# RubensBenevides/Point-Cloud-Registration-with-Global-Refinement

Measured on AMD Instinct MI355X. Metric: point-cloud pairs registered/sec (200k pts, 3 GICP scales), higher is better.
Workload: dtype f32 points+search, f64 normal equations (SURVEY 8a fp column)

## Files before the change

point-cloud-registration-with-global-refinement_amd/csrc/pcr_api.hip:

```cpp
#include <cmath>
#include <cstring>
#include <cstdlib>
#include <cstdio>
#include <atomic>
#include <mutex>
#include <thread>
#include <vector>
#include "pcr_octree.h"

extern "C" int pcr_version(void) { return 220; }

PcrOptions &pcr_options() {
    static PcrOptions o;
    static std::once_flag once;
    std::call_once(once, []() {
        if (const char *e = getenv("PCR_KNN_WAVE")) o.knn_wave = atoi(e);
        if (const char *e = getenv("PCR_KNNW_BUDGET")) o.knnw_budget = atoi(e);
        if (const char *e = getenv("PCR_FENCE_PREP")) o.fence_prep = atoi(e);
        if (getenv("PCR_ICP_VERIFY")) o.icp_verify = 1;
        if (const char *e = getenv("PCR_SPFH_FLOAT64")) o.spfh_float64 = atoi(e);
        if (const char *e = getenv("PCR_RADIUS_LIST_SELECT")) o.radius_list_select = atoi(e);
        if (const char *e = getenv("PCR_FEATNN_MUTUAL")) o.featnn_mutual = atoi(e);
        if (const char *e = getenv("PCR_ICP_SCALES")) o.icp_scales = atoi(e);
        if (const char *e = getenv("PCR_SEARCH_SORT_QUERIES")) o.search_sort_queries = atoi(e);
        if (const char *e = getenv("PCR_FPS_FORM")) o.fps_form = atoi(e);
        if (const char *e = getenv("PCR_FPS_WGS")) o.fps_wgs = atoi(e);
        if (const char *e = getenv("PCR_FPS_TIMEOUT")) o.fps_timeout = atoi(e);
    });
    return o;
}
PcrCounters &pcr_counters() { static PcrCounters c; return c; }
extern "C" long long pcr_counter(const char *name, int reset) {
    if (!name) return -1;
    PcrCounters &c = pcr_counters();
    std::atomic<long long> *v = !strcmp(name, "fgr_group_barrier_timeouts") ? &c.fgr_group_barrier_timeouts : !strcmp(name, "fgr_group_pool_overflows") ? &c.fgr_group_pool_overflows
                               : !strcmp(name, "fgr_group_pairs_redone_alone") ? &c.fgr_group_pairs_redone_alone : nullptr;
    if (!v) return -1;
    return reset ? v->exchange(0) : v->load();
}
extern "C" int pcr_set_option(const char *name, long long value) {
    if (!name) return PCR_EINVAL;
    PcrOptions &o = pcr_options();
    if (!strcmp(name, "knn_wave")) { o.knn_wave = (int)value; return PCR_OK; }
    if (!strcmp(name, "knnw_budget")) { o.knnw_budget = (int)value; return PCR_OK; }
    if (!strcmp(name, "fence_prep")) { o.fence_prep = (int)value; return PCR_OK; }
    if (!strcmp(name, "icp_verify")) { o.icp_verify = (int)value; return PCR_OK; }
    if (!strcmp(name, "spfh_float64")) { o.spfh_float64 = (int)value; return PCR_OK; }
    if (!strcmp(name, "radius_list_select")) { o.radius_list_select = (int)value; return PCR_OK; }
    if (!strcmp(name, "arena_poison")) { o.arena_poison = (int)value; return PCR_OK; }
    if (!strcmp(name, "featnn_mutual")) { o.featnn_mutual = (int)value; return PCR_OK; }
    if (!strcmp(name, "icp_scales")) { o.icp_scales = (int)value; return PCR_OK; }
    if (!strcmp(name, "search_sort_queries")) { o.search_sort_queries = (int)value; return PCR_OK; }
    if (!strcmp(name, "fps_form")) { o.fps_form = (int)value; return PCR_OK; }
    if (!strcmp(name, "fps_wgs")) { o.fps_wgs = (int)value; return PCR_OK; }
    if (!strcmp(name, "fps_timeout")) { o.fps_timeout = (int)value; return PCR_OK; }
    return PCR_EINVAL;
}

extern "C" int pcr_create(int device, pcr_context **out) {
    if (!out) return PCR_EINVAL;
    *out = nullptr;
    int count = 0;
    if (hipGetDeviceCount(&count) != hipSuccess || count <= 0) return PCR_EHIP;
    if (device < 0 || device >= count) return PCR_EINVAL;
    if (hipSetDevice(device) != hipSuccess) return PCR_EHIP;
    pcr_context *ctx = new pcr_context();
    ctx->device = device;
    for (int i = 0; i < 2; i++)
        if (hipEventCreateWithFlags(&ctx->side_ev[i], hipEventDisableTiming) != hipSuccess) { delete ctx; return PCR_EHIP; }
    for (int i = 0; i < 8; i++)
        if (hipEventCreateWithFlags(&ctx->lane_ev[i], hipEventDisableTiming) != hipSuccess) { delete ctx; return PCR_EHIP; }
    ctx->pinned_cap = 1 << 16;
    if (hipHostMalloc((void **)&ctx->pinned, ctx->pinned_cap, hipHostMallocDefault) != hipSuccess) { delete ctx; return PCR_EHIP; }
    for (int i = 0; i < 2; i++)
        if (hipEventCreateWithFlags(&ctx->ev[i], hipEventDisableTiming) != hipSuccess) { delete ctx; return PCR_EHIP; }
    for (int i = 0; i < 2; i++)
        if (hipEventCreateWithFlags(&ctx->fence_ev[i], hipEventDisableTiming) != hipSuccess) { delete ctx; return PCR_EHIP; }
    ctx->fence_default = true;
    *out = ctx;
    return PCR_OK;
}

extern "C" int pcr_destroy(pcr_context *ctx) {
    if (!ctx) return PCR_OK;
    (void)hipSetDevice(ctx->device);
    if (ctx->stream) (void)hipStreamSynchronize(ctx->stream);
    if (ctx->arena) (void)hipFree(ctx->arena);
    if (ctx->aux) (void)hipFree(ctx->aux);
    if (ctx->icp_group_dev) (void)hipFree(ctx->icp_group_dev);
    if (ctx->icp_group_host) (void)hipHostFree(ctx->icp_group_host);
    if (ctx->desc_dev) (void)hipFree(ctx->desc_dev);
    if (ctx->desc_host) (void)hipHostFree(ctx->desc_host);
    if (ctx->pinned) (void)hipHostFree(ctx->pinned);
    for (int i = 0; i < 2; i++) if (ctx->ev[i]) (void)hipEventDestroy(ctx->ev[i]);
    for (int i = 0; i < 2; i++) if (ctx->fence_ev[i]) (void)hipEventDestroy(ctx->fence_ev[i]);
    for (hipEvent_t e : ctx->prof_events) (void)hipEventDestroy(e);
    for (auto &g : ctx->icp_graphs) { (void)hipGraphExecDestroy(g.exec); if (g.graph) (void)hipGraphDestroy(g.graph); }
    if (ctx->own_stream) (void)hipStreamDestroy(ctx->own_stream);
    if (ctx->side_stream) { (void)hipStreamSynchronize(ctx->side_stream); (void)hipStreamDestroy(ctx->side_stream); }
    if (ctx->side_stream2) { (void)hipStreamSynchronize(ctx->side_stream2); (void)hipStreamDestroy(ctx->side_stream2); }
    for (int i = 0; i < 2; i++) if (ctx->side_ev[i]) (void)hipEventDestroy(ctx->side_ev[i]);
    for (int i = 0; i < 8; i++) if (ctx->lane_ev[i]) (void)hipEventDestroy(ctx->lane_ev[i]);
    delete ctx;
    return PCR_OK;
}

extern "C" int pcr_set_stream(pcr_context *ctx, void *s) {
    if (!ctx) return PCR_EINVAL;
    if (ctx->stream) (void)hipStreamSynchronize(ctx->stream);
    ctx->stream = s ? (hipStream_t)s : ctx->own_stream;
    ctx->fence_default = (s == nullptr);
    return PCR_OK;
}
static void use_private_stream(pcr_context *ctx) {
    if (ctx->stream) (void)hipStreamSynchronize(ctx->stream);
    ctx->stream = ctx->own_stream;
    ctx->fence_default = false;
}

extern "C" int pcr_profile_enable(pcr_context *ctx, int on) {
    if (!ctx) return PCR_EINVAL;
    ctx->profiling = on ? 1 : 0;
    return PCR_OK;
}
extern "C" int pcr_profile_read(pcr_context *ctx, double *out16, int reset) {
    if (!ctx || !out16) return PCR_EINVAL;
    for (int i = 0; i < 16; i++) { out16[i] = ctx->prof[i]; if (reset) ctx->prof[i] = 0; }
    return PCR_OK;
}

extern "C" const char *pcr_last_error(const pcr_context *ctx) { return ctx ? ctx->err.c_str() : "null context"; }

int pcr_arena_reserve(pcr_context *ctx, size_t bytes) {
    ctx->arena_off = 0;
    if (const int poison = pcr_options().arena_poison.load(std::memory_order_relaxed)) {
        if (ctx->arena) { PCR_HIP_CHECK(ctx, hipDeviceSynchronize()); PCR_HIP_CHECK(ctx, hipMemset(ctx->arena, poison & 0xff, ctx->arena_cap)); }
    }
    if (bytes <= ctx->arena_cap) return PCR_OK;
// ... 1191 lines not shown
```

point-cloud-registration-with-global-refinement_amd/csrc/pcr_cloud.hip:

```cpp
#include <cstdlib>
#include <cstring>
#include <cstdio>
#include <vector>
#include "pcr_octree.h"

#define BS 256

struct BoundsArgs { const float *xyz; int64_t n; float *part; float *out6; int nb; };
struct OpBoundsPartial : PcrOp<BoundsArgs, BS> {
    __device__ static inline void run(const BoundsArgs &a) {
        if ((int)blockIdx.x >= a.nb) return;
        float mn[3] = {3.4e38f, 3.4e38f, 3.4e38f}, mx[3] = {-3.4e38f, -3.4e38f, -3.4e38f};
        for (int64_t i = blockIdx.x * (int64_t)BS + threadIdx.x; i < a.n; i += (int64_t)a.nb * BS) {
            float x = a.xyz[i * 3], y = a.xyz[i * 3 + 1], z = a.xyz[i * 3 + 2];
            mn[0] = fminf(mn[0], x); mn[1] = fminf(mn[1], y); mn[2] = fminf(mn[2], z);
            mx[0] = fmaxf(mx[0], x); mx[1] = fmaxf(mx[1], y); mx[2] = fmaxf(mx[2], z);
        }
        __shared__ float s[BS / PCR_WAVE][6];
        const int lane = threadIdx.x & 63, w = threadIdx.x >> 6;
#pragma unroll
        for (int d = 0; d < 3; d++) { mn[d] = pcr_wave_min(mn[d]); mx[d] = pcr_wave_max(mx[d]); }
        if (lane == 0) { for (int d = 0; d < 3; d++) { s[w][d] = mn[d]; s[w][3 + d] = mx[d]; } }
        __syncthreads();
        if (threadIdx.x < 6) {
// ... 1375 lines not shown
                if ((ci & hm) == (ipre & hm)) atomicAdd(&dig[ob][(ci >> sh) & 255u], 1u);
            });
            __builtin_amdgcn_fence(__ATOMIC_RELEASE, "workgroup"); __builtin_amdgcn_wave_barrier(); __builtin_amdgcn_fence(__ATOMIC_ACQUIRE, "workgroup");
            if (act) {
                int cum = 0, b = 0;
                for (; b < 255; b++) { const int h = (int)dig[ob][b]; if (cum + h >= r2) break; cum += h; }
                r2 -= cum;
                ipre = (ipre & hm) | ((unsigned long long)b << sh);
            }
            __builtin_amdgcn_wave_barrier();
        }
        int cnt = 0;
        auto write = [&](int first, int count) {
            for (int base = first; base < first + count; base += OCT) {
                const int idx = base + ol;
                bool take = false;
                if (fix && idx < first + count) {
                    const float4 p = a.t.pts[idx];
                    const float d2 = pcr_d2(p.x - q.x, p.y - q.y, p.z - q.z);
                    if (d2 < a.r2f && d2 <= hi) {
                        if (d2 < lo || all_band) take = true;
                        else {
                            const unsigned long long kk = key_of(p);
                            take = kk < kpre || (kk == kpre && (all_ties || (unsigned long long)a.perm[idx] <= ipre));
                        }
                    }
                }
                const unsigned mask = (unsigned)(__ballot(take) >> (oct * 8)) & 0xffu;
                const int pos = cnt + __builtin_popcount(mask & ((1u << ol) - 1u));
                if (take && pos < a.k) row[pos] = idx;
                cnt += __builtin_popcount(mask);
            }
        };
        oct_search_group(a.t, m, gstk[threadIdx.x >> 6], fix, leaf0, q.x, q.y, q.z, [&]() { return wb; }, write,
                         [](int, int) { return false; }, ol);
    }
}
struct OpRadiusFix : PcrOp<RadListArgs, KNN_BS> { __device__ static inline void run(const RadListArgs &a) { d_radius_fix(a); } };
int pcr_dev_radius_lists_batch(pcr_context *ctx, const DevCloud *const *cs, const uint32_t *const *perms, int count, int k, double radius, int32_t *const *idx, int32_t *const *cnt) {
    if (count < 1) return PCR_OK;
    if (count > PCR_MAX_GROUP_BATCH) { ctx->err = "radius list batch size"; return PCR_EINVAL; }
    if (!(radius > 0) || k < 1 || k > 200) { ctx->err = "radius lists: radius <= 0 or k outside 1..200"; return PCR_EINVAL; }
    std::vector<RadListArgs> ra; std::vector<KnnArgs> ka; std::vector<int> caps;
    int *counts = arena<int>(ctx, count);
    if (!counts) return PCR_ENOMEM;
    PCR_HIP_CHECK(ctx, hipMemsetAsync(counts, 0, sizeof(int) * (size_t)count, ctx->stream));
    int mc = 0;
    for (int c = 0; c < count; c++) {
        if (cs[c]->cap <= 0) continue;
        RadListArgs r;
        r.t = oct_view(cs[c]); r.n_ptr = cs[c]->n; r.r2f = (float)(radius * radius); r.k = k; r.idx = idx[c]; r.cnt = cnt[c];
        r.over_list = arena<int>(ctx, (size_t)cs[c]->cap / OCT + 1); r.over_count = counts + c;
        r.select = pcr_options().radius_list_select.load(std::memory_order_relaxed); r.perm = perms[c];
        if (!r.over_list) return PCR_ENOMEM;
        ra.push_back(r);
        KnnArgs a; std::memset(&a, 0, sizeof a);
        a.t = r.t; a.n_ptr = cs[c]->n; a.k = k;
        knn_radius(a, PCR_SEARCH_HYBRID, radius);
        a.r2cap_f = r.r2f;
        a.dbg_idx = idx[c]; a.dbg_d2 = nullptr; a.dbg_cnt = nullptr; a.seed_span = -1;
        a.hard_piece = 1; a.hard_list = r.over_list; a.hard_count = r.over_count;
        ka.push_back(a); caps.push_back(cs[c]->cap);
        mc = cs[c]->cap > mc ? cs[c]->cap : mc;
    }
    const int m = (int)ra.size();
    if (m == 0) return PCR_OK;
    PCR_TRY(PCR_BATCH_LAUNCH(ctx, OpRadiusList, ra.data(), m, dim3((unsigned)(((size_t)mc * OCT + KNN_BS - 1) / KNN_BS), m)));
    int lg = mc / (OCT * (KNN_BS / 64) * 4); lg = lg < 8 ? 8 : (lg > 2048 ? 2048 : lg);
    const dim3 grid(lg, m);
    PCR_TRY((launch_knn_octet_slots<KNN_MODE_DEBUG, true>(ctx, ka.data(), m, k, grid)));
    PCR_TRY(PCR_BATCH_LAUNCH(ctx, OpRadiusFix, ra.data(), m, grid));
    return PCR_OK;
}

struct NflArgs {
    const float4 *pts; const int *n_ptr;
    const int32_t *lidx;
    const uint8_t *keep; const int *pos;
    int k_list, k_nrm;
    const float4 *prior; float4 *normals;
    uint8_t *todo; int *todo_count;
    int *piece_list, *piece_count;
};
__device__ static inline void d_normals_from_lists(const NflArgs &a) {
    const int n = *a.n_ptr;
    const int ol = threadIdx.x & 7, oct_id = (threadIdx.x & 63) >> 3;
    const int base = (blockIdx.x * (KNN_BS / 64) + (threadIdx.x >> 6)) * 64;
    if (base >= n) return;
    double my_cu[9] = {0, 0, 0, 0, 0, 0, 0, 0, 0}, my_c = 0;
    bool my_exact = false; int my_j = 0;
    bool piece_todo = false;
#pragma unroll 1
    for (int r = 0; r < OCT; r++) {
        const int i = base + oct_id * OCT + r;
        const bool act = i < n && a.keep[i];
        int id[4]; float d[4]; bool ok[4]; float4 pn[4];
        int lc = 0, vc = 0;
        const float4 qp = a.pts[act ? i : 0];
#pragma unroll
        for (int s = 0; s < 4; s++) {
            const int slot = ol + OCT * s;
            id[s] = (act && slot < a.k_list) ? a.lidx[(size_t)i * 32 + slot] : -1;
            pn[s] = a.pts[id[s] >= 0 ? id[s] : 0];
            d[s] = id[s] >= 0 ? pcr_d2(pn[s].x - qp.x, pn[s].y - qp.y, pn[s].z - qp.z) : -1.0f;
            ok[s] = id[s] >= 0 && a.keep[id[s]];
            lc += id[s] >= 0 ? 1 : 0; vc += ok[s] ? 1 : 0;
        }
        lc = pcr_octet_sum_i(lc); vc = pcr_octet_sum_i(vc);
        const bool exact = act && (vc >= a.k_nrm || lc < a.k_list);
        const int j = act ? a.pos[i] : 0;
        if (act && ol == 0) {
            a.todo[j] = exact ? 0 : 1;
            if (!exact) atomicAdd(a.todo_count, 1);
        }
        piece_todo = piece_todo || (act && !exact);
        int excess = exact ? vc - a.k_nrm : 0;
        while (__ballot(excess > 0) != 0ull) {
            float m = -1.0f; int ms = 0;
#pragma unroll
            for (int s = 0; s < 4; s++) if (ok[s] && d[s] > m) { m = d[s]; ms = s; }
            const float om = pcr_octet_max(m);
            const int ml = __builtin_ctz((uint32_t)(__ballot(m == om) >> (threadIdx.x & 56)) & 0xffu);
            const bool hit = excess > 0 && ol == ml;
#pragma unroll
            for (int s = 0; s < 4; s++) ok[s] = ok[s] && !(hit && s == ms);
            excess -= excess > 0 ? 1 : 0;
        }
        double cu[9] = {0, 0, 0, 0, 0, 0, 0, 0, 0}, c = 0;
#pragma unroll
        for (int s = 0; s < 4; s++) {
            if (exact && ok[s]) {
                const float4 p = pn[s];
                const double x = p.x, y = p.y, z = p.z;
                cu[0] += x; cu[1] += y; cu[2] += z;
                cu[3] += x * x; cu[4] += x * y; cu[5] += x * z; cu[6] += y * y; cu[7] += y * z; cu[8] += z * z;
                c += 1.0;
            }
        }
#pragma unroll
        for (int t = 0; t < 9; t++) cu[t] = pcr_octet_sum(cu[t]);
        c = pcr_octet_sum(c);
        if (ol == r) {
            my_exact = exact; my_j = j; my_c = c;
#pragma unroll
            for (int t = 0; t < 9; t++) my_cu[t] = cu[t];
        }
    }
    if (a.piece_list && piece_todo && ol == 0) a.piece_list[atomicAdd(a.piece_count, 1)] = base + oct_id * OCT;
    if (!my_exact) return;
    double myC[6] = {1, 0, 0, 1, 0, 1};
    if (my_c >= 3.0) {
#pragma unroll
        for (int t = 0; t < 9; t++) my_cu[t] = my_cu[t] / my_c;
        myC[0] = my_cu[3] - my_cu[0] * my_cu[0]; myC[1] = my_cu[4] - my_cu[0] * my_cu[1]; myC[2] = my_cu[5] - my_cu[0] * my_cu[2];
        myC[3] = my_cu[6] - my_cu[1] * my_cu[1]; myC[4] = my_cu[7] - my_cu[1] * my_cu[2]; myC[5] = my_cu[8] - my_cu[2] * my_cu[2];
    }
    double nv[3];
    d_fast_eigen3x3(myC, nv);
    const double nn = sqrt(nv[0] * nv[0] + nv[1] * nv[1] + nv[2] * nv[2]);
    double px = 0, py = 0, pz = 0;
    if (a.prior) { const float4 pr = a.prior[my_j]; px = pr.x; py = pr.y; pz = pr.z; }
    if (nn == 0.0 || !(nn == nn)) { if (a.prior) { nv[0] = px; nv[1] = py; nv[2] = pz; } else { nv[0] = 0; nv[1] = 0; nv[2] = 1; } }
    if (a.prior && nv[0] * px + nv[1] * py + nv[2] * pz < 0.0) { nv[0] = -nv[0]; nv[1] = -nv[1]; nv[2] = -nv[2]; }
    a.normals[my_j] = make_float4((float)nv[0], (float)nv[1], (float)nv[2], 0.0f);
}

struct OpNormalsFromLists : PcrOp<NflArgs, KNN_BS> { __device__ static inline void run(const NflArgs &a) { d_normals_from_lists(a); } };

#define SOR_STAT_BLOCKS 128
struct SorStatArgs { const double *avg; const int *n_ptr; double std_ratio; double *out3; double *partials ; unsigned int *ticket; };
__device__ static inline void d_sor_stats(const SorStatArgs &aa) {
    const double *__restrict__ avg = aa.avg; const int *__restrict__ n_ptr = aa.n_ptr; const double std_ratio = aa.std_ratio;
    double *__restrict__ out3 = aa.out3; double *__restrict__ partials = aa.partials; unsigned int *__restrict__ ticket = aa.ticket;
    __shared__ double red[16][3];
    __shared__ double rows[SOR_STAT_BLOCKS * 3];
    __shared__ int is_last;
    const int n = *n_ptr, t = threadIdx.x;
    double c = 0.0;
    for (int i = 0; i < n && i < 64; i++) { const double v = avg[i]; if (v > 0) { c = v; break; } }
    double a = 0, b = 0, cnt = 0;
    for (int i = blockIdx.x * 256 + t; i < n; i += gridDim.x * 256) { const double v = avg[i]; if (v > 0) { const double d = v - c; a += d; b += d * d; cnt += 1.0; } }
    a = pcr_row16_sum(a); b = pcr_row16_sum(b); cnt = pcr_row16_sum(cnt);
    if ((t & 15) == 0) { red[t >> 4][0] = a; red[t >> 4][1] = b; red[t >> 4][2] = cnt; }
    __syncthreads();
    if (t < 3) {
        double s = 0;
        for (int r = 0; r < 16; r++) s += red[r][t];
        __hip_atomic_store(&partials[blockIdx.x * 4 + t], s, __ATOMIC_RELAXED, __HIP_MEMORY_SCOPE_AGENT);
    }
    asm volatile("s_waitcnt vmcnt(0)" ::: "memory");
    __syncthreads();
    if (t == 0) is_last = __hip_atomic_fetch_add(ticket, 1u, __ATOMIC_RELAXED, __HIP_MEMORY_SCOPE_AGENT) == gridDim.x - 1;
    __syncthreads();
    if (!is_last) return;
    for (int e = t; e < 3 * (int)gridDim.x; e += 256) {
        const double *p = partials + (e / 3) * 4 + (e % 3);
        double v;
        asm volatile("global_load_dwordx2 %0, %1, off sc0 sc1\n\ts_waitcnt vmcnt(0)" : "=&v"(v) : "v"(p) : "memory");
        rows[e] = v;
    }
    __syncthreads();
    if (t == 0) {
        double sa = 0, sb = 0, sc = 0;
        for (int r = 0; r < (int)gridDim.x; r++) { sa += rows[3 * r]; sb += rows[3 * r + 1]; sc += rows[3 * r + 2]; }
        const double valid = sc;
        const double mean = valid > 0 ? c + sa / valid : 0.0;
        const double var = valid > 1 ? (sb - sa * sa / valid) / (valid - 1.0) : 0.0;
        const double sd = sqrt(var > 0 ? var : 0.0);
        out3[0] = mean; out3[1] = sd; out3[2] = valid > 0 ? mean + std_ratio * sd : -1.0;
        *ticket = 0u;
    }
}
struct OpSorStats : PcrOp<SorStatArgs, 256> { __device__ static inline void run(const SorStatArgs &a) { d_sor_stats(a); } };

struct CompactArgs {
    const float4 *pts, *nrm; const uint8_t *flags; const int *pos; const int *n_ptr; float4 *out_pts, *out_nrm;
    const uint64_t *keys; uint64_t *out_keys; int *cnt_in_out, *cnt_kept_out; const int *kept_n;
};
__device__ static inline void d_compact_cloud(const CompactArgs &a) {
    const int i = blockIdx.x * BS + threadIdx.x;
    if (i == 0) { if (a.cnt_in_out) *a.cnt_in_out = *a.n_ptr; if (a.cnt_kept_out) *a.cnt_kept_out = *a.kept_n; }
    if (i >= *a.n_ptr || !a.flags[i]) return;
    const int o = a.pos[i];
    a.out_pts[o] = a.pts[i];
    a.out_keys[o] = a.keys[i];
    if (a.nrm && a.out_nrm) a.out_nrm[o] = a.nrm[i];
}
struct OpCompactCloud : PcrOp<CompactArgs, BS> { __device__ static inline void run(const CompactArgs &a) { d_compact_cloud(a); } };

struct SorProblem {
    const DevCloud *in; DevCloud *out; uint8_t *keep_sorted; double *avg_sorted; const float4 *prior_out; uint8_t *todo_out; int *todo_count;
    int *cnt_in_out, *cnt_kept_out;
};
static int sor_batch(pcr_context *ctx, SorProblem *pr, int count, int nb_neighbors, double std_ratio, int normal_k, bool fallback_here) {
    if (nb_neighbors < 1 || !(std_ratio > 0.0)) { ctx->err = "nb_neighbors < 1 or std_ratio <= 0"; return PCR_EINVAL; }
    if (count < 1 || count > PCR_MAX_GROUP_BATCH) { ctx->err = "SOR batch size"; return PCR_EINVAL; }
    std::vector<KnnArgs> kbv((size_t)count), fbv((size_t)count); std::vector<SorStatArgs> sbv((size_t)count); std::vector<ScanArgs> cbv((size_t)count);
    std::vector<CompactArgs> mbv((size_t)count); std::vector<NflArgs> nbv((size_t)count);
    std::memset(kbv.data(), 0, sizeof(KnnArgs) * (size_t)count); std::memset(fbv.data(), 0, sizeof(KnnArgs) * (size_t)count);
    std::memset(sbv.data(), 0, sizeof(SorStatArgs) * (size_t)count); std::memset(cbv.data(), 0, sizeof(ScanArgs) * (size_t)count);
    std::memset(mbv.data(), 0, sizeof(CompactArgs) * (size_t)count); std::memset(nbv.data(), 0, sizeof(NflArgs) * (size_t)count);
    KnnArgs *const kb = kbv.data(), *const fb = fbv.data(); SorStatArgs *const sb = sbv.data(); ScanArgs *const cb = cbv.data();
    CompactArgs *const mb = mbv.data(); NflArgs *const nb_ = nbv.data();
    std::vector<int> capsv((size_t)count); int *caps = capsv.data(); int m = 0;
    bool any_todo = false, fuse_all = true;
    int *piece_counts = (fallback_here && normal_k > 0 && normal_k <= 32) ? arena<int>(ctx, count) : nullptr;
    if (piece_counts) PCR_HIP_CHECK(ctx, hipMemsetAsync(piece_counts, 0, sizeof(int) * (size_t)count, ctx->stream));
    for (int k = 0; k < count; k++) {
        SorProblem &q = pr[k];
        const DevCloud *in = q.in; DevCloud *out = q.out;
        for (int d = 0; d < 3; d++) { out->key_org[d] = in->key_org[d]; out->key_unit[d] = in->key_unit[d]; }
        out->voxel_lattice = in->voxel_lattice;
        if (in->cap <= 0) { PCR_HIP_CHECK(ctx, hipMemsetAsync(out->n, 0, sizeof(int), ctx->stream)); continue; }
        double *avg = q.avg_sorted ? q.avg_sorted : arena<double>(ctx, in->cap);
        double *stats3 = arena<double>(ctx, 4);
        double *stat_partials = arena<double>(ctx, SOR_STAT_BLOCKS * 4);
        unsigned int *stat_ticket = arena<unsigned int>(ctx, 1);
        uint8_t *flags = q.keep_sorted ? q.keep_sorted : arena<uint8_t>(ctx, in->cap);
        int *pos = arena<int>(ctx, in->cap);
        if (!avg || !stats3 || !stat_partials || !stat_ticket || !flags || !pos) return PCR_ENOMEM;
        const bool fuse = normal_k > 0 && q.todo_out && nb_neighbors <= 32 && normal_k <= nb_neighbors;
        const int pitch = nb_neighbors <= 32 ? 32 : 64;
        int32_t *lidx = (fuse || nb_neighbors <= 64) ? arena<int32_t>(ctx, (size_t)in->cap * pitch) : nullptr;
        if ((fuse || nb_neighbors <= 64) && !lidx) return PCR_ENOMEM;
        KnnArgs &a = kb[m];
        a.t = oct_view(in); a.n_ptr = in->n; a.k = nb_neighbors; a.avg = avg; a.list_idx = lidx; a.list_pitch = pitch;
        a.zero_a = (int *)stat_ticket; a.zero_b = (fuse && q.todo_out) ? q.todo_count : nullptr;
        a.seed_span = -1;
        knn_radius(a, PCR_SEARCH_KNN, 0);
        sb[m] = SorStatArgs{avg, in->n, std_ratio, stats3, stat_partials, stat_ticket};
        PCR_TRY(scan_args(ctx, &cb[m], flags, in->n, in->cap, pos, out->n, FlagSrc{nullptr, avg, stats3}));
        mb[m] = CompactArgs{in->pts, in->nrm, flags, pos, in->n, out->pts, out->nrm, in->keys, out->keys, q.cnt_in_out, q.cnt_kept_out, out->n};
        if (q.todo_out) {
            any_todo = true;
            if (fuse) {
                NflArgs &f = nb_[m];
                f.pts = in->pts; f.n_ptr = in->n; f.lidx = lidx; f.keep = flags; f.pos = pos; f.k_list = nb_neighbors; f.k_nrm = normal_k;
                f.prior = q.prior_out; f.normals = out->nrm_final; f.todo = q.todo_out; f.todo_count = q.todo_count;
            } else {
                fuse_all = false;
                PCR_HIP_CHECK(ctx, hipMemsetAsync(q.todo_out, 1, (size_t)in->cap, ctx->stream));
            }
            if (fallback_here && normal_k > 0) {
                KnnArgs &b = fb[m];
                b.t = oct_view(in); b.n_ptr = in->n; b.k = normal_k; b.prior = q.prior_out; b.normals = out->nrm_final; b.todo = fuse ? q.todo_out : nullptr;
                b.keep = flags; b.pos = pos; b.seed_span = -1;
                knn_radius(b, PCR_SEARCH_KNN, 0);
                if (fuse && piece_counts) {
                    int *pl = arena<int>(ctx, (size_t)in->cap / OCT + 1);
                    if (!pl) return PCR_ENOMEM;
                    nb_[m].piece_list = pl; nb_[m].piece_count = piece_counts + m;
                    b.hard_list = pl; b.hard_count = piece_counts + m; b.hard_piece = 1;
                }
            }
        } else fuse_all = false;
        caps[m] = in->cap;
        m++;
    }
    if (m == 0) return PCR_OK;
    int mc = 0;
    for (int k = 0; k < m; k++) mc = caps[k] > mc ? caps[k] : mc;
    if (m > 1 && nb_neighbors > 32) { ctx->err = "batched SOR: nb_neighbors must be <= 32"; return PCR_EINVAL; }
    PCR_TRY(launch_knn_batch<KNN_MODE_SOR>(ctx, kb, caps, m));
    PCR_TRY(PCR_BATCH_LAUNCH(ctx, OpSorStats, sb, m, dim3(SOR_STAT_BLOCKS, m)));
    PCR_TRY(flag_scan_batch(ctx, cb, m));
    PCR_TRY(PCR_BATCH_LAUNCH(ctx, OpCompactCloud, mb, m, dim3((mc + BS - 1) / BS, m)));
    if (any_todo) {
        if (fuse_all) PCR_TRY(PCR_BATCH_LAUNCH(ctx, OpNormalsFromLists, nb_, m, dim3((unsigned)(((size_t)mc + KNN_BS - 1) / KNN_BS), m)));
        else for (int k = 0; k < m; k++) if (nb_[k].pts) PCR_TRY(PCR_BATCH_LAUNCH(ctx, OpNormalsFromLists, nb_ + k, 1, dim3((unsigned)(((size_t)caps[k] + KNN_BS - 1) / KNN_BS))));
        if (fallback_here && normal_k > 0) {
            bool listed = fuse_all && piece_counts != nullptr;
            for (int k = 0; k < m; k++) listed = listed && fb[k].hard_list != nullptr;
            if (listed) {
                using Op = OpKnn<KNN_MODE_NORMALS, 4, true>;
                PCR_TRY(PCR_BATCH_LAUNCH(ctx, Op, fb, m, dim3(knn_list_grid(mc), m)));
            } else if (normal_k <= 32) PCR_TRY(launch_knn_batch<KNN_MODE_NORMALS>(ctx, fb, caps, m));
            else PCR_TRY(launch_knn_each<KNN_MODE_NORMALS>(ctx, fb, caps, m));
        }
    }
    return PCR_OK;
}

int pcr_dev_sor(pcr_context *ctx, const DevCloud *in, int nb_neighbors, double std_ratio, DevCloud *out, uint8_t *keep_sorted, double *avg_sorted,
                int normal_k, const float4 *prior_out, uint8_t *todo_out, int *todo_count, int *cnt_in_out, int *cnt_kept_out, bool fallback_here) {
    ArenaMark mark(ctx);
    SorProblem p{in, out, keep_sorted, avg_sorted, prior_out, todo_out, todo_count, cnt_in_out, cnt_kept_out};
    return sor_batch(ctx, &p, 1, nb_neighbors, std_ratio, normal_k, fallback_here);
}
int pcr_dev_sor_batch(pcr_context *ctx, const DevCloud *const *ins, DevCloud *const *outs, int count, int nb_neighbors, double std_ratio, int normal_k,
                      const float4 *const *priors, uint8_t *const *todos, int *const *todo_counts, int *const *cnt_in, int *const *cnt_kept, bool fallback_here) {
    if (count > PCR_MAX_GROUP_BATCH) { ctx->err = "SOR batch size"; return PCR_EINVAL; }
    std::vector<SorProblem> pv((size_t)(count > 0 ? count : 1)); SorProblem *p = pv.data();
    for (int k = 0; k < count; k++) p[k] = SorProblem{ins[k], outs[k], nullptr, nullptr, priors ? priors[k] : nullptr, todos[k], todo_counts[k], cnt_in ? cnt_in[k] : nullptr, cnt_kept ? cnt_kept[k] : nullptr};
    return sor_batch(ctx, p, count, nb_neighbors, std_ratio, normal_k, fallback_here);
}
int pcr_dev_normals_batch(pcr_context *ctx, DevCloud *const *cs, int count, int search_kind, int knn, double radius, const float4 *const *priors, float4 *const *normals_out,
                          const uint8_t *const *todos) {
    if (search_kind != PCR_SEARCH_KNN && search_kind != PCR_SEARCH_HYBRID) { ctx->err = "normals batch: KNN or Hybrid search"; return PCR_EINVAL; }
    if (search_kind == PCR_SEARCH_HYBRID && !(radius > 0)) { ctx->err = "radius <= 0"; return PCR_EINVAL; }
    if (knn < 1) { ctx->err = "knn < 1"; return PCR_EINVAL; }
    if (count > PCR_MAX_GROUP_BATCH) { ctx->err = "normals batch size"; return PCR_EINVAL; }
    std::vector<KnnArgs> bv((size_t)(count > 0 ? count : 1)); std::memset(bv.data(), 0, sizeof(KnnArgs) * bv.size());
    KnnArgs *const b = bv.data(); std::vector<int> capsv((size_t)(count > 0 ? count : 1)); int *caps = capsv.data(); int m = 0;
    for (int k = 0; k < count; k++) {
        if (cs[k]->cap <= 0) continue;
        KnnArgs &a = b[m];
        a.t = oct_view(cs[k]); a.n_ptr = cs[k]->n; a.k = knn; a.prior = priors ? priors[k] : nullptr; a.normals = normals_out[k]; a.todo = todos ? todos[k] : nullptr; a.seed_span = -1;
        knn_radius(a, search_kind, radius);
        caps[m++] = cs[k]->cap;
    }
    if (m == 0) return PCR_OK;
    if (knn <= 32) return launch_knn_batch<KNN_MODE_NORMALS>(ctx, b, caps, m);
    return launch_knn_each<KNN_MODE_NORMALS>(ctx, b, caps, m);
}
int pcr_dev_knn_lists_batch(pcr_context *ctx, const DevCloud *const *cs, int count, int k, double radius, int32_t *const *idx, float *const *d2) {
    if (count < 1) return PCR_OK;
    if (count > PCR_MAX_GROUP_BATCH) { ctx->err = "k-NN list batch size"; return PCR_EINVAL; }
    std::vector<KnnArgs> av((size_t)count); std::memset(av.data(), 0, sizeof(KnnArgs) * av.size());
    std::vector<int> caps((size_t)count); int m = 0;
    for (int c = 0; c < count; c++) {
        if (cs[c]->cap <= 0) continue;
        KnnArgs &a = av[m];
        a.t = oct_view(cs[c]); a.n_ptr = cs[c]->n; a.k = k;
        knn_radius(a, radius > 0 ? PCR_SEARCH_HYBRID : PCR_SEARCH_KNN, radius);
        if (radius > 0) a.r2cap_f = (float)(radius * radius);
        a.dbg_idx = idx[c]; a.dbg_d2 = d2[c]; a.dbg_cnt = nullptr;
        caps[m++] = cs[c]->cap;
    }
    if (m == 0) return PCR_OK;
    return launch_knn_octet_batch<KNN_MODE_DEBUG>(ctx, av.data(), caps.data(), m);
}
int pcr_dev_flag_scan_batch(pcr_context *ctx, int count, uint8_t *const *flags, const int *const *n_ptr, const int *n_cap, int *const *pos, int *const *total_dev) {
    if (count < 1) return PCR_OK;
    std::vector<ScanArgs> a((size_t)count);
    for (int c = 0; c < count; c++) PCR_TRY(scan_args(ctx, &a[c], flags[c], n_ptr ? n_ptr[c] : nullptr, n_cap[c], pos[c], total_dev[c], FlagSrc{nullptr, nullptr, nullptr}));
    return flag_scan_batch(ctx, a.data(), count);
}

int pcr_dev_normals(pcr_context *ctx, DevCloud *c, int search_kind, int knn, double radius, const float4 *prior, float4 *normals_out, float *cov6_out,
                    const uint8_t *todo) {
    if (search_kind == PCR_SEARCH_RADIUS) {
        if (!(radius > 0)) { ctx->err = "radius <= 0"; return PCR_EINVAL; }
        if (c->cap <= 0) return PCR_OK;
        RadArgs r;
        r.t = oct_view(c); r.n_ptr = c->n; r.r2 = radius * radius; r.r2f = pcr_wide_r2f(r.r2);
        r.prior = prior; r.normals = normals_out; r.cov6 = cov6_out;
        PCR_LAUNCH(ctx, k_radius_moments, dim3((unsigned)(((size_t)c->cap * OCT + KNN_BS - 1) / KNN_BS)), dim3(KNN_BS), 0, ctx->stream, r);
        return PCR_OK;
    }
    if (knn < 1) { ctx->err = "knn < 1"; return PCR_EINVAL; }
    if (search_kind == PCR_SEARCH_HYBRID && !(radius > 0)) { ctx->err = "radius <= 0"; return PCR_EINVAL; }
    KnnArgs a = {};
// ... 10 lines not shown
```

point-cloud-registration-with-global-refinement_amd/csrc/pcr_internal.h:

```cpp
#pragma once
#include <hip/hip_runtime.h>
#include <stdint.h>
#include <string>
#include <mutex>
#include <cstring>
#include <vector>
#include <atomic>
#include "../../include/pcr_hip.h"

struct PcrOptions { std::atomic<int> knn_wave{-1}, knnw_budget{80}, fence_prep{0}, icp_verify{0}, spfh_float64{0}, radius_list_select{1}, arena_poison{0}, featnn_mutual{1}, icp_scales{1}, search_sort_queries{-1}, fps_form{-1}, fps_wgs{0}, fps_timeout{-1}; };
PcrOptions &pcr_options();
struct PcrCounters { std::atomic<long long> fgr_group_barrier_timeouts{0}, fgr_group_pool_overflows{0}, fgr_group_pairs_redone_alone{0}; };
PcrCounters &pcr_counters();
#define PCR_GROUP_FORMS_MAX_POINTS 400000


struct IcpGraph {
    std::string key;
    hipGraphExec_t exec = nullptr;
    hipGraph_t graph = nullptr;
    std::vector<hipGraphNode_t> nodes;
    std::string baked;
};

struct pcr_context {
    int device = 0;
    hipStream_t stream = nullptr;
    hipStream_t own_stream = nullptr;
    hipStream_t side_stream = nullptr;
    hipStream_t side_stream2 = nullptr;
    hipEvent_t side_ev[2] = {nullptr, nullptr};
    hipEvent_t lane_ev[8] = {};
    char *arena = nullptr;
    size_t arena_cap = 0, arena_off = 0;
    char *aux = nullptr;
    size_t aux_cap = 0;
    char *desc_host = nullptr, *desc_dev = nullptr;
    size_t desc_cap = 0, desc_off = 0;
    char *icp_group_dev = nullptr, *icp_group_host = nullptr;
    char *pinned = nullptr;
    size_t pinned_cap = 0;
    hipEvent_t ev[2] = {nullptr, nullptr};
    int profiling = 0;
    double prof[16] = {0, 0, 0, 0, 0, 0, 0, 0, 0, 0, 0, 0, 0, 0, 0, 0};
    std::vector<hipEvent_t> prof_events;
    std::vector<IcpGraph> icp_graphs;
    std::string err;
    bool fence_default = false;
    hipEvent_t fence_ev[2] = {nullptr, nullptr};
    hipError_t launch_err = hipSuccess;
    const char *launch_file = nullptr; int launch_line = 0;
    bool group_forms = false;
    bool octet_only = false;
};

int pcr_enter(pcr_context *ctx);
int pcr_leave(pcr_context *ctx, int rc);
template <class F> static inline int pcr_api_call(pcr_context *ctx, F &&body) {
    const int rc = pcr_enter(ctx);
    if (rc != PCR_OK) return rc;
    return pcr_leave(ctx, body());
}

template <class... KArgs, class... Args>
static inline void pcr_launch(pcr_context *ctx, const char *file, int line, void (*kernel)(KArgs...), dim3 grid, dim3 block, size_t shmem,
                              hipStream_t stream, Args &&...args) {
    hipLaunchKernelGGL(kernel, grid, block, shmem, stream, static_cast<KArgs>(args)...);
    const hipError_t e = hipGetLastError();
    if (e != hipSuccess && ctx->launch_err == hipSuccess) { ctx->launch_err = e; ctx->launch_file = file; ctx->launch_line = line; }
}
#define PCR_LAUNCH(ctx, ...) pcr_launch(ctx, __FILE__, __LINE__, __VA_ARGS__)

#define PCR_HIP_CHECK(ctx, expr)                                                                   \
    do {                                                                                           \
        hipError_t _e = (expr);                                                                    \
        if (_e != hipSuccess) {                                                                    \
            (ctx)->err = std::string(#expr) + ": " + hipGetErrorString(_e);                        \
            return PCR_EHIP;                                                                       \
        }                                                                                          \
    } while (0)

#define PCR_TRY(expr)                                                                              \
    do {                                                                                           \
        int _rc = (expr);                                                                          \
        if (_rc != PCR_OK) return _rc;                                                             \
    } while (0)

template <class A> static inline const A *pcr_desc_upload(pcr_context *ctx, const A *host, int count) {
    const size_t bytes = (sizeof(A) * (size_t)count + 255) & ~(size_t)255;
    if (!ctx->desc_host) {
        ctx->desc_cap = 8u << 20;
        if (hipHostMalloc((void **)&ctx->desc_host, ctx->desc_cap, hipHostMallocDefault) != hipSuccess) { ctx->desc_host = nullptr; ctx->err = "hipHostMalloc(descriptors)"; return nullptr; }
        if (hipMalloc((void **)&ctx->desc_dev, ctx->desc_cap) != hipSuccess) { ctx->desc_dev = nullptr; ctx->err = "hipMalloc(descriptors)"; return nullptr; }
// ... 160 lines not shown
```

Before: 660.2.

## Add lane-per-point normals-from-lists kernel with branchless top-k trimming

Adds a new normals-from-lists kernel form in which each lane owns one point and reads its 32 neighbor slots directly. The old form had eight lanes cooperate per point with iterative octet max-reductions. Excess neighbors are trimmed with a per-lane sorting-chain selection instead of ballot loops, and moments are accumulated with masked loads and a fixed summation order through LDS. It is enabled by default through a new nfl_form option. The cost is higher register and LDS pressure per lane, and possibly different rounding order.

```diff
diff --git a/point-cloud-registration-with-global-refinement_amd/csrc/pcr_api.hip b/point-cloud-registration-with-global-refinement_amd/csrc/pcr_api.hip
--- a/point-cloud-registration-with-global-refinement_amd/csrc/pcr_api.hip
+++ b/point-cloud-registration-with-global-refinement_amd/csrc/pcr_api.hip
@@ -26,6 +26,7 @@
         if (const char *e = getenv("PCR_FPS_FORM")) o.fps_form = atoi(e);
         if (const char *e = getenv("PCR_FPS_WGS")) o.fps_wgs = atoi(e);
         if (const char *e = getenv("PCR_FPS_TIMEOUT")) o.fps_timeout = atoi(e);
+        if (const char *e = getenv("PCR_NFL_FORM")) o.nfl_form = atoi(e);
     });
     return o;
 }
@@ -54,6 +55,7 @@
     if (!strcmp(name, "fps_form")) { o.fps_form = (int)value; return PCR_OK; }
     if (!strcmp(name, "fps_wgs")) { o.fps_wgs = (int)value; return PCR_OK; }
     if (!strcmp(name, "fps_timeout")) { o.fps_timeout = (int)value; return PCR_OK; }
+    if (!strcmp(name, "nfl_form")) { o.nfl_form = (int)value; return PCR_OK; }
     return PCR_EINVAL;
 }
 
diff --git a/point-cloud-registration-with-global-refinement_amd/csrc/pcr_cloud.hip b/point-cloud-registration-with-global-refinement_amd/csrc/pcr_cloud.hip
--- a/point-cloud-registration-with-global-refinement_amd/csrc/pcr_cloud.hip
+++ b/point-cloud-registration-with-global-refinement_amd/csrc/pcr_cloud.hip
@@ -1481,6 +1481,29 @@
     uint8_t *todo; int *todo_count;
     int *piece_list, *piece_count;
 };
+__device__ static inline void nfl_add_moments(double (&cu)[9], float px, float py, float pz) {
+    const double x = px, y = py, z = pz;
+    cu[0] += x; cu[1] += y; cu[2] += z;
+    cu[3] += x * x; cu[4] += x * y; cu[5] += x * z; cu[6] += y * y; cu[7] += y * z; cu[8] += z * z;
+}
+__device__ static inline void nfl_solve_and_store(const NflArgs &a, double (&my_cu)[9], double my_c, int my_j) {
+    double myC[6] = {1, 0, 0, 1, 0, 1};
+    if (my_c >= 3.0) {
+#pragma unroll
+        for (int t = 0; t < 9; t++) my_cu[t] = my_cu[t] / my_c;
+        myC[0] = my_cu[3] - my_cu[0] * my_cu[0]; myC[1] = my_cu[4] - my_cu[0] * my_cu[1]; myC[2] = my_cu[5] - my_cu[0] * my_cu[2];
+        myC[3] = my_cu[6] - my_cu[1] * my_cu[1]; myC[4] = my_cu[7] - my_cu[1] * my_cu[2]; myC[5] = my_cu[8] - my_cu[2] * my_cu[2];
+    }
+    double nv[3];
+    d_fast_eigen3x3(myC, nv);
+    const double nn = sqrt(nv[0] * nv[0] + nv[1] * nv[1] + nv[2] * nv[2]);
+    double px = 0, py = 0, pz = 0;
+    if (a.prior) { const float4 pr = a.prior[my_j]; px = pr.x; py = pr.y; pz = pr.z; }
+    if (nn == 0.0 || !(nn == nn)) { if (a.prior) { nv[0] = px; nv[1] = py; nv[2] = pz; } else { nv[0] = 0; nv[1] = 0; nv[2] = 1; } }
+    if (a.prior && nv[0] * px + nv[1] * py + nv[2] * pz < 0.0) { nv[0] = -nv[0]; nv[1] = -nv[1]; nv[2] = -nv[2]; }
+    a.normals[my_j] = make_float4((float)nv[0], (float)nv[1], (float)nv[2], 0.0f);
+}
+
 __device__ static inline void d_normals_from_lists(const NflArgs &a) {
     const int n = *a.n_ptr;
     const int ol = threadIdx.x & 7, oct_id = (threadIdx.x & 63) >> 3;
@@ -1529,10 +1552,7 @@
 #pragma unroll
         for (int s = 0; s < 4; s++) {
             if (exact && ok[s]) {
-                const float4 p = pn[s];
-                const double x = p.x, y = p.y, z = p.z;
-                cu[0] += x; cu[1] += y; cu[2] += z;
-                cu[3] += x * x; cu[4] += x * y; cu[5] += x * z; cu[6] += y * y; cu[7] += y * z; cu[8] += z * z;
+                nfl_add_moments(cu, pn[s].x, pn[s].y, pn[s].z);
                 c += 1.0;
             }
         }
@@ -1547,24 +1567,159 @@
     }
     if (a.piece_list && piece_todo && ol == 0) a.piece_list[atomicAdd(a.piece_count, 1)] = base + oct_id * OCT;
     if (!my_exact) return;
-    double myC[6] = {1, 0, 0, 1, 0, 1};
-    if (my_c >= 3.0) {
-#pragma unroll
-        for (int t = 0; t < 9; t++) my_cu[t] = my_cu[t] / my_c;
-        myC[0] = my_cu[3] - my_cu[0] * my_cu[0]; myC[1] = my_cu[4] - my_cu[0] * my_cu[1]; myC[2] = my_cu[5] - my_cu[0] * my_cu[2];
-        myC[3] = my_cu[6] - my_cu[1] * my_cu[1]; myC[4] = my_cu[7] - my_cu[1] * my_cu[2]; myC[5] = my_cu[8] - my_cu[2] * my_cu[2];
-    }
-    double nv[3];
-    d_fast_eigen3x3(myC, nv);
-    const double nn = sqrt(nv[0] * nv[0] + nv[1] * nv[1] + nv[2] * nv[2]);
-    double px = 0, py = 0, pz = 0;
-    if (a.prior) { const float4 pr = a.prior[my_j]; px = pr.x; py = pr.y; pz = pr.z; }
-    if (nn == 0.0 || !(nn == nn)) { if (a.prior) { nv[0] = px; nv[1] = py; nv[2] = pz; } else { nv[0] = 0; nv[1] = 0; nv[2] = 1; } }
-    if (a.prior && nv[0] * px + nv[1] * py + nv[2] * pz < 0.0) { nv[0] = -nv[0]; nv[1] = -nv[1]; nv[2] = -nv[2]; }
-    a.normals[my_j] = make_float4((float)nv[0], (float)nv[1], (float)nv[2], 0.0f);
-}
+    nfl_solve_and_store(a, my_cu, my_c, my_j);
+}
+
+#define NFL_GLOBAL __attribute__((address_space(1)))
+typedef int nfl_int4 __attribute__((ext_vector_type(4)));
+__device__ static inline const NFL_GLOBAL float *nfl_point(const float4 *pts, int id) {
+    return (const NFL_GLOBAL float *)((const NFL_GLOBAL char *)pts + ((unsigned)id << 4));
+}
+template <int CH>
+__device__ static inline void d_normals_from_lists_lane(const NflArgs &a) {
+    __shared__ double quad0_lds[9][KNN_BS];
+    volatile __attribute__((address_space(3))) double *quad0 = (volatile __attribute__((address_space(3))) double *)&quad0_lds[0][threadIdx.x];
+    const float4 *__restrict__ pts = a.pts; const uint8_t *__restrict__ keep = a.keep;
+    const int k_list = a.k_list, k_nrm = a.k_nrm;
+    const int n = *a.n_ptr;
+    const int lane = threadIdx.x & 63;
+    const int base = (blockIdx.x * (KNN_BS / 64) + (threadIdx.x >> 6)) * 64;
+    if (base >= n) return;
+    const int i = base + lane;
+    const bool act = i < n && keep[i < n ? i : 0] != 0;
+    const int32_t *__restrict__ row = a.lidx + (size_t)(act ? i : 0) * 32;
+    const float4 qp = pts[act ? i : 0];
+    const int klim = act ? k_list : 0;
+    int d[32];
+    int lc = -32; unsigned okm = 0;
+    nfl_int4 v4 = ((const NFL_GLOBAL nfl_int4 *)row)[0];
+#pragma unroll
+    for (int q = 0; q < 8; q++) {
+        nfl_int4 nx = ((const NFL_GLOBAL nfl_int4 *)row)[q < 7 ? q + 1 : 7];
+        const int v[4] = {v4.x, v4.y, v4.z, v4.w};
+        int id[4]; float px[4], py[4], pz[4]; unsigned kb[4];
+#pragma unroll
+        for (int e = 0; e < 4; e++) {
+            id[e] = 4 * q + e < klim ? v[e] : -1;
+            const int idc = max(id[e], 0);
+            const NFL_GLOBAL float *pn = nfl_point(pts, idc);
+            px[e] = pn[0]; py[e] = pn[1]; pz[e] = pn[2];
+            kb[e] = *((const NFL_GLOBAL uint8_t *)keep + (unsigned)idc);
+        }
+        asm volatile("" : "+v"(px[0]), "+v"(py[0]), "+v"(pz[0]), "+v"(kb[0]), "+v"(px[1]), "+v"(py[1]), "+v"(pz[1]), "+v"(kb[1]),
+                          "+v"(px[2]), "+v"(py[2]), "+v"(pz[2]), "+v"(kb[2]), "+v"(px[3]), "+v"(py[3]), "+v"(pz[3]), "+v"(kb[3]),
+                          "+v"(nx.x), "+v"(nx.y), "+v"(nx.z), "+v"(nx.w));
+#pragma unroll
+        for (int e = 0; e < 4; e++) {
+            const int slot = 4 * q + e, bit = 4 * (slot & 7) + (slot >> 3);
+            const float dd = pcr_d2(px[e] - qp.x, py[e] - qp.y, pz[e] - qp.z);
+            const unsigned ok = (unsigned)min((int)kb[e], 1) & ~(unsigned)(id[e] >> 31);
+            d[slot] = ok ? __float_as_int(dd) : __float_as_int(-1.0f);
+            lc -= id[e] >> 31; okm |= ok << bit;
+        }
+        asm volatile("" : "+v"(d[4 * q]), "+v"(d[4 * q + 1]), "+v"(d[4 * q + 2]), "+v"(d[4 * q + 3]), "+v"(okm), "+v"(lc));
+        v4 = nx;
+    }
+    const int vc = __popc(okm);
+    const bool exact = act && (vc >= k_nrm || -lc < k_list);
+    const int j = act ? a.pos[i] : 0;
+    if (act) a.todo[j] = exact ? 0 : 1;
+    const unsigned long long tb = __ballot(act && !exact);
+    if (tb != 0ull && lane == 0) atomicAdd(a.todo_count, __popcll(tb));
+    if (a.piece_list && (lane & 7) == 0 && ((tb >> lane) & 0xffull) != 0ull) a.piece_list[atomicAdd(a.piece_count, 1)] = base + lane;
+    const int excess = exact ? vc - k_nrm : 0;
+    unsigned dropm = 0;
+    if (__ballot(excess > 0) != 0ull) {
+        int ch[CH];
+#pragma unroll
+        for (int t = 0; t < CH; t++) ch[t] = __float_as_int(-1.0f);
+#pragma unroll
+        for (int s = 0; s < 32; s++) {
+#pragma unroll
+            for (int t = CH - 1; t >= 1; t--) ch[t] = max(min(ch[t - 1], ch[t]), min(max(ch[t - 1], ch[t]), d[s]));
+            ch[0] = max(ch[0], d[s]);
+        }
+        int thr = ch[0];
+#pragma unroll
+        for (int t = 1; t < CH; t++) thr = excess > t ? ch[t] : thr;
+        thr = excess > 0 ? thr : 0x7fffffff;
+        unsigned gtm = 0, eqm = 0;
+#pragma unroll
+        for (int s = 0; s < 32; s++) {
+            const int bit = 4 * (s & 7) + (s >> 3);
+            gtm |= (d[s] > thr ? 1u : 0u) << bit; eqm |= (d[s] == thr ? 1u : 0u) << bit;
+            if ((s & 3) == 3) __builtin_amdgcn_sched_barrier(0);
+        }
+        int need = excess > 0 ? excess - __popc(gtm) : 0;
+        unsigned eq_kept = eqm;
+        while (__ballot(need > 0) != 0ull) {
+            if (need > 0) { eq_kept &= eq_kept - 1u; need--; }
+        }
+        dropm = gtm | (eqm & ~eq_kept);
+    }
+    const unsigned keptm = exact ? okm & ~dropm : 0u;
+    const NFL_GLOBAL int32_t *row2 = (const NFL_GLOBAL int32_t *)row;
+    asm volatile("" : "+v"(row2));
+    double pair[9] = {0, 0, 0, 0, 0, 0, 0, 0, 0}, lone[9] = {0, 0, 0, 0, 0, 0, 0, 0, 0};
+#pragma unroll 1
+    for (int r = 0; r < OCT; r++) {
+        double P[9] = {0, 0, 0, 0, 0, 0, 0, 0, 0};
+        const int kr = (int)(keptm >> (4 * r));
+        int id4[4]; float px[4], py[4], pz[4];
+#pragma unroll
+        for (int s = 0; s < 4; s++) id4[s] = row2[r + OCT * s];
+        asm volatile("" : "+v"(id4[0]), "+v"(id4[1]), "+v"(id4[2]), "+v"(id4[3]));
+#pragma unroll
+        for (int s = 0; s < 4; s++) {
+            const NFL_GLOBAL float *pn = nfl_point(pts, id4[s] & __builtin_amdgcn_sbfe(kr, s, 1));
+            px[s] = pn[0]; py[s] = pn[1]; pz[s] = pn[2];
+        }
+        asm volatile("" : "+v"(px[0]), "+v"(py[0]), "+v"(pz[0]), "+v"(px[1]), "+v"(py[1]), "+v"(pz[1]),
+                          "+v"(px[2]), "+v"(py[2]), "+v"(pz[2]), "+v"(px[3]), "+v"(py[3]), "+v"(pz[3]));
+#pragma unroll
+        for (int s = 0; s < 4; s++) {
+            int m = kr;
+            asm volatile("" : "+v"(m));
+            m = __builtin_amdgcn_sbfe(m, s, 1);
+            nfl_add_moments(P, __int_as_float(__float_as_int(px[s]) & m), __int_as_float(__float_as_int(py[s]) & m), __int_as_float(__float_as_int(pz[s]) & m));
+        }
+        if ((r & 1) == 0) {
+#pragma unroll
+            for (int t = 0; t < 9; t++) lone[t] = P[t];
+        } else if ((r & 2) == 0) {
+#pragma unroll
+            for (int t = 0; t < 9; t++) pair[t] = lone[t] + P[t];
+        } else {
+#pragma unroll
+            for (int t = 0; t < 9; t++) pair[t] = pair[t] + (lone[t] + P[t]);
+            if (r == 3) {
+#pragma unroll
+                for (int t = 0; t < 9; t++) quad0[t * KNN_BS] = pair[t];
+            }
+        }
+    }
+    double my_cu[9];
+#pragma unroll
+    for (int t = 0; t < 9; t++) my_cu[t] = quad0[t * KNN_BS] + pair[t];
+    if (!exact) return;
+    int my_j = j;
+    asm volatile("" : "+v"(my_j));
+    nfl_solve_and_store(a, my_cu, (double)__popc(keptm), my_j);
+}
+static int nfl_lane_chain(int k_list, int k_nrm) { return k_list - k_nrm <= 10 ? 10 : 31; }
 
 struct OpNormalsFromLists : PcrOp<NflArgs, KNN_BS> { __device__ static inline void run(const NflArgs &a) { d_normals_from_lists(a); } };
+template <int CH> struct OpNormalsFromListsLane : PcrOp<NflArgs, KNN_BS> {
+    static constexpr int kWavesMin = 6, kWavesMax = 8;
+    __device__ static inline void run(const NflArgs &a) { [[clang::always_inline]] d_normals_from_lists_lane<CH>(a); }
+};
+static int launch_normals_from_lists(pcr_context *ctx, const NflArgs *args, int count, dim3 grid) {
+    if (pcr_options().nfl_form.load(std::memory_order_relaxed) == 0) return PCR_BATCH_LAUNCH(ctx, OpNormalsFromLists, args, count, grid);
+    int chain = 10;
+    for (int k = 0; k < count; k++) if (args[k].pts && nfl_lane_chain(args[k].k_list, args[k].k_nrm) > chain) chain = 31;
+    if (chain == 10) return PCR_BATCH_LAUNCH(ctx, OpNormalsFromListsLane<10>, args, count, grid);
+    return PCR_BATCH_LAUNCH(ctx, OpNormalsFromListsLane<31>, args, count, grid);
+}
 
 #define SOR_STAT_BLOCKS 128
 struct SorStatArgs { const double *avg; const int *n_ptr; double std_ratio; double *out3; double *partials ; unsigned int *ticket; };
@@ -1705,8 +1860,8 @@
     PCR_TRY(flag_scan_batch(ctx, cb, m));
     PCR_TRY(PCR_BATCH_LAUNCH(ctx, OpCompactCloud, mb, m, dim3((mc + BS - 1) / BS, m)));
     if (any_todo) {
-        if (fuse_all) PCR_TRY(PCR_BATCH_LAUNCH(ctx, OpNormalsFromLists, nb_, m, dim3((unsigned)(((size_t)mc + KNN_BS - 1) / KNN_BS), m)));
-        else for (int k = 0; k < m; k++) if (nb_[k].pts) PCR_TRY(PCR_BATCH_LAUNCH(ctx, OpNormalsFromLists, nb_ + k, 1, dim3((unsigned)(((size_t)caps[k] + KNN_BS - 1) / KNN_BS))));
+        if (fuse_all) PCR_TRY(launch_normals_from_lists(ctx, nb_, m, dim3((unsigned)(((size_t)mc + KNN_BS - 1) / KNN_BS), m)));
+        else for (int k = 0; k < m; k++) if (nb_[k].pts) PCR_TRY(launch_normals_from_lists(ctx, nb_ + k, 1, dim3((unsigned)(((size_t)caps[k] + KNN_BS - 1) / KNN_BS))));
         if (fallback_here && normal_k > 0) {
             bool listed = fuse_all && piece_counts != nullptr;
             for (int k = 0; k < m; k++) listed = listed && fb[k].hard_list != nullptr;
diff --git a/point-cloud-registration-with-global-refinement_amd/csrc/pcr_internal.h b/point-cloud-registration-with-global-refinement_amd/csrc/pcr_internal.h
--- a/point-cloud-registration-with-global-refinement_amd/csrc/pcr_internal.h
+++ b/point-cloud-registration-with-global-refinement_amd/csrc/pcr_internal.h
@@ -8,7 +8,7 @@
 #include <atomic>
 #include "../../include/pcr_hip.h"
 
-struct PcrOptions { std::atomic<int> knn_wave{-1}, knnw_budget{80}, fence_prep{0}, icp_verify{0}, spfh_float64{0}, radius_list_select{1}, arena_poison{0}, featnn_mutual{1}, icp_scales{1}, search_sort_queries{-1}, fps_form{-1}, fps_wgs{0}, fps_timeout{-1}; };
+struct PcrOptions { std::atomic<int> knn_wave{-1}, knnw_budget{80}, fence_prep{0}, icp_verify{0}, spfh_float64{0}, radius_list_select{1}, arena_poison{0}, featnn_mutual{1}, icp_scales{1}, search_sort_queries{-1}, fps_form{-1}, fps_wgs{0}, fps_timeout{-1}, nfl_form{1}; };
 PcrOptions &pcr_options();
 struct PcrCounters { std::atomic<long long> fgr_group_barrier_timeouts{0}, fgr_group_pool_overflows{0}, fgr_group_pairs_redone_alone{0}; };
 PcrCounters &pcr_counters();
```

After: 685.7, median of 6. 3.9% higher.
